# dohlee/rosettafold-pytorch

Hardware: AMD Instinct MI355X
Metric: residues/sec forward (L=256, N=128) (higher is better)
Workload: dtype bf16; 1 GPU; BASELINE.json configs[1]: bsz=4/GPU, n_seq=128, L=256, d_msa=384, d_pair=288, 8+5 blocks, 4 encoder layers, random-init weights; global_batch=4, parallelism=batch-sharded x1 (replicated weights), launch=one hipGraph replay per step (validation + input copy outside the graph)

## Files before the change

### include/rfmi.h

```cpp
#ifndef RFMI_H
#define RFMI_H
#include <stdint.h>

#ifdef __cplusplus
extern "C" {
#endif

#define RF_F32 0
#define RF_BF16 1
#define RF_F16 2
#define RF_F32X3 3

#define RF_EINVAL (-1)
#define RF_EALIGN (-2)

#define RF_ACT_NONE 0
#define RF_ACT_RELU 1
#define RF_ACT_ELU 2
#define RF_ACT_RELU_EPS 3
#define RF_ACT_LEAKY 4
#define RF_ACT_BLOCK_LN32 5

#define RF_BIAS_NONE 0
#define RF_BIAS_COL 1
// ... 93 lines not shown

int rf_outer_product_ln_linear(const void* xt, const void* yt, const void* wprime, const float* s, const float* c, float* out,
                               int B, int L, int N, int P, int Dout, float eps, const float* ln2_gamma, const float* ln2_beta,
                               float ln2_eps, void* y, int64_t y_ld, void* stream);

int rf_poswise(const void* q0, int q0_dtype, int64_t q0_ld, const void* k, int64_t k_ld, int k_col0, int k_hstride,
               int dlen, float* w, void* q_scale, int64_t qs_ld, int qs_col0, int qs_dh, int dtype, int B, int N, int L,
               int H, float scale, float qscale, void* stream);

int rf_weighted_msa_sum(const void* x, int dtype, const float* w, float* y, int64_t y_ld, int B, int N, int L, int D,
                        void* stream);

int64_t rf_instnorm_ws_bytes(int B, int64_t HW, int C);
int rf_instnorm_stats(const void* x, int x_dtype, void* sums , int B, int64_t HW, int C, void* workspace,
                      int64_t ws_bytes, void* stream);
int rf_instnorm_apply(const void* x, int x_dtype, const void* sums, const float* gamma, const float* beta, float eps,
                      const float* residual, int act, void* y, int y_dtype, void* y2, int y2_dtype, int B, int64_t HW,
                      int C, void* stream);

int rf_instnorm_mean(const void* sums, float* mean, int B, int64_t HW, int C, void* stream);
int64_t rf_channel_mean_ws_bytes(int B, int64_t HW, int C);
int rf_channel_mean(const float* x, float* mean, int B, int64_t HW, int C, void* workspace, int64_t ws_bytes, void* stream);
int rf_sample_mean(const void* x, int x_dtype, float* mean, int B, int64_t R, int C, int nsample, void* stream);
int rf_center_apply(const float* x, const float* mean, void* y, int y_dtype, int B, int64_t HW, int C, void* stream);
int rf_center_rows(float* x, float* mean, int B, int R, int C, void* stream);
int rf_fold_mean(const float* w, int64_t ldw, int k0, int K, int nseg, int64_t seg_stride, int sum_seg, const float* mean,
                 const float* bias, float* out, int B, int N, void* stream);
int rf_conv3x3_border_fix(void* y, int y_dtype, const float* taps, int B, int H, int W, int C, int dilation, int edges,
                          void* stream);

// ... 126 lines not shown
```

### rosettafold-pytorch_amd/_lib.py

```python
import ctypes as C
import os

import torch

_HERE = os.path.dirname(os.path.abspath(__file__))
LIB_PATH = os.environ.get("RFMI_LIB") or os.path.join(_HERE, "librfmi.so")

RF_F32, RF_BF16, RF_F16 = 0, 1, 2
RF_F32X3 = 3
ACT_NONE, ACT_RELU, ACT_ELU, ACT_RELU_EPS, ACT_LEAKY, ACT_BLOCK_LN32 = 0, 1, 2, 3, 4, 5
BIAS_NONE, BIAS_COL, BIAS_ROW = 0, 1, 2
AMODE_PLAIN, AMODE_CONV3X3 = 0, 1

i32, i64, f32, vp = C.c_int32, C.c_int64, C.c_float, C.c_void_p
u64 = C.c_uint64


class GemmDesc(C.Structure):
    _fields_ = [
        ("M", i32), ("N", i32), ("K", i32),
        ("nb0", i32), ("nb1", i32), ("nb2", i32),
        ("ab_dtype", i32), ("c_dtype", i32), ("kc", i32), ("a_mode", i32),
        ("a_rc", i32), ("b_rc", i32), ("c_rc", i32), ("c_cc", i32),
        ("a_bs", i64 * 3), ("a_ro", i64), ("a_ri", i64), ("a_ko", i64),
# ... 24 lines not shown
    "rf_tied_attention": [vp, vp, vp, C.POINTER(I64x4), C.POINTER(I64x4), vp, C.POINTER(I64x3), f32, vp, vp, i64, vp,
                          C.POINTER(I64x4), i32, i32, i32, i32, i32, vp, i64, vp],
    "rf_tied_softmax_ld": [vp, vp, i32, i64, vp, i64, i32, i32, i32, vp],
    "rf_tied_logits_ld": [vp, vp, C.POINTER(I64x4), vp, C.POINTER(I64x3), f32, vp, i64, vp, i64, i32, i32, i32, i32, i32, vp,
                          i64, vp],
    "rf_tied_av_ld": [vp, i64, vp, C.POINTER(I64x4), vp, C.POINTER(I64x4), i32, i32, i32, i32, i32, vp],
    "rf_tied_attention_ld": [vp, vp, vp, C.POINTER(I64x4), C.POINTER(I64x4), vp, C.POINTER(I64x3), f32, vp, i64, vp, i64, vp,
                             C.POINTER(I64x4), i32, i32, i32, i32, i32, vp, i64, vp],
    "rf_ffn_fused": [vp, i64, vp, vp, vp, vp, i64, vp, i64, vp, i64, vp, vp, f32, i64, i32, i32, vp],
    "rf_outer_product_ln_linear": [vp, vp, vp, vp, vp, vp, i32, i32, i32, i32, i32, f32, vp, vp, f32, vp, i64, vp],
    "rf_poswise_collapsed": [vp, vp, vp, i32, i32, i32, i32, i32, f32, vp],
    "rf_poswise": [vp, i32, i64, vp, i64, i32, i32, i32, vp, vp, i64, i32, i32, i32, i32, i32, i32, i32, f32, f32, vp],
    "rf_weighted_msa_sum": [vp, i32, vp, vp, i64, i32, i32, i32, i32, vp],
    "rf_instnorm_ws_bytes": [i32, i64, i32],
    "rf_instnorm_stats": [vp, i32, vp, i32, i64, i32, vp, i64, vp],
    "rf_instnorm_apply": [vp, i32, vp, vp, vp, f32, vp, i32, vp, i32, vp, i32, i32, i64, i32, vp],
    "rf_instnorm_mean": [vp, vp, i32, i64, i32, vp],
    "rf_channel_mean_ws_bytes": [i32, i64, i32],
    "rf_channel_mean": [vp, vp, i32, i64, i32, vp, i64, vp],
    "rf_sample_mean": [vp, i32, vp, i32, i64, i32, i32, vp],
    "rf_center_apply": [vp, vp, vp, i32, i32, i64, i32, vp],
    "rf_center_rows": [vp, vp, i32, i32, i32, vp],
    "rf_fold_mean": [vp, i64, i32, i32, i32, i64, i32, vp, vp, vp, i32, i32, vp],
    "rf_conv3x3_border_fix": [vp, i32, vp, i32, i32, i32, i32, i32, i32, vp],
    "rf_msa_embed": [vp, vp, vp, vp, vp, vp, i32, i32, i32, i32, vp],
    "rf_pair_embed": [vp, vp, vp, vp, vp, vp, vp, vp, i32, i32, i32, vp],
    "rf_copy4d": [vp, i32, C.POINTER(I64x4), vp, i32, C.POINTER(I64x4), C.POINTER(I64x4), vp],
    "rf_axpby": [vp, i32, f32, vp, i32, f32, vp, i32, i64, vp],
    "rf_favor_softmax_features": [vp, vp, C.POINTER(I64x4), i32, i32, vp, i32, i64, i32, i32, i32, i32, i32, i32, f32, vp],
    "rf_favor_attention": [vp, vp, vp, C.POINTER(I64x4), C.POINTER(I64x3), i32, i32, i32, i32, i32, i32, i32, i32, i32, i32, f32, vp],
# ... 109 lines not shown
```

### rosettafold-pytorch_amd/csrc/common.h

```cpp
#pragma once
#include <hip/hip_runtime.h>
#include <stdint.h>
#include <stdlib.h>

#include "rfmi.h"

typedef __attribute__((ext_vector_type(8))) short h16x8;
typedef __attribute__((ext_vector_type(4))) short h16x4;
typedef __attribute__((ext_vector_type(4))) float f32x4;
typedef unsigned short h16_t;
typedef __attribute__((ext_vector_type(2))) float rf_f32x2;

#define RF_WAVE 64

#ifdef RF_H16_IS_F16
#define RF_H16 RF_F16
#define RF_H16_ONE2 0x3C003C00u
typedef __attribute__((ext_vector_type(2))) _Float16 rf_h16x2;
typedef __attribute__((ext_vector_type(8))) _Float16 rf_h16x8n;
__device__ __forceinline__ float h2f(h16_t u) { return (float)__builtin_bit_cast(_Float16, u); }
__device__ __forceinline__ h16_t f2h(float x) { return __builtin_bit_cast(h16_t, (_Float16)x); }
__device__ __forceinline__ f32x4 rf_mfma16(h16x8 a, h16x8 b, f32x4 c, int, int, int) {
  return __builtin_amdgcn_mfma_f32_16x16x32_f16(__builtin_bit_cast(rf_h16x8n, a), __builtin_bit_cast(rf_h16x8n, b), c, 0, 0, 0);
}
// ... 119 lines not shown
  *out = v ? atoi(v) : 0;
  return 0;
}
#else
#define RF_DBG(x) 0
static inline int rf_dbg_env(const char* name, int* out) {
  *out = 0;
  return getenv(name) ? RF_EINVAL : 0;
}
#endif

static inline bool rf_env_flag(const char* name) { return getenv(name) != nullptr; }

int rf_gemm_fast_try(const rf_gemm_desc& d, int64_t batch, int* rc, void* stream);
int rf_gemm_wreg_try(const rf_gemm_desc& d, int64_t batch, int* rc, void* stream);
int rf_conv288_try(const rf_gemm_desc& d, int64_t batch, int* rc, void* stream);
void rf_gemm_fast_set_stamps(void* buf);
```

### rosettafold-pytorch_amd/csrc/conv288.hip

```cpp
#include <type_traits>

#include "common.h"

static __device__ __attribute__((aligned(16))) unsigned int g_conv_zero16[4];

struct Conv288P {
  const h16_t* x;
  const h16_t* w;
  const float* bias;
  h16_t* y;
  int B, H, W, dil;
  int tpr;
  int nt_store;
};

__global__ __launch_bounds__(512) void conv3x3_c288_kernel(const Conv288P p) {
  constexpr int C = 288, BM = 256, BN = 288;
  constexpr int WGN = 2, TM = 64, TN = 144, WM = 4, WN = 9;
  constexpr int A_PIECES = 17, B_PIECES = 18;
  constexpr int A_BYTES = A_PIECES * 1024, B_BYTES = B_PIECES * 1024;
  constexpr int SSTEP = A_BYTES + 3 * B_BYTES;
  constexpr int NPIECES = A_PIECES + 3 * B_PIECES;
  constexpr int PW = (NPIECES + 7) / 8;
  constexpr int NSS = 27;
  extern __shared__ __attribute__((aligned(16))) char smem[];
  const int tid = threadIdx.x, lane = tid & 63;
  const int wave = __builtin_amdgcn_readfirstlane(tid >> 6);
  const int wm = wave / WGN, wn = wave % WGN;
  const int fr = lane & 15, fq = lane >> 4;
// ... 77 lines not shown
    __builtin_amdgcn_s_barrier();
#pragma unroll
    for (int t = 0; t < PW; ++t) CONV_DMA(t)
    const unsigned sbase = (unsigned)((ss & 1) * SSTEP);
#include "conv288_schedule.inc"
  }
#undef CONV_RD
#undef CONV_RDA
#undef CONV_DMA

  __syncthreads();
  constexpr int PITCH = TN * 2 + 16;
  constexpr int CPR = TN * 2 / 16;
  constexpr int NIT = 32 * CPR / 64;
  char* const strip = smem + wave * (32 * PITCH);
  h16_t* const ytile = p.y + ((int64_t)row * p.W + j0) * C;
#pragma unroll
  for (int ip = 0; ip < 2; ++ip) {
#pragma unroll
    for (int ih = 0; ih < 2; ++ih)
#pragma unroll
      for (int j = 0; j < WN; ++j) {
        const f32x4 a = acc[ip * 2 + ih][j];
        uint2 o;
        o.x = rf_pack2_h16(a[0], a[1]);
        o.y = rf_pack2_h16(a[2], a[3]);
        *(uint2*)(strip + (ih * 16 + fr) * PITCH + (j * 16 + 4 * fq) * 2) = o;
      }
    asm volatile("" ::: "memory");
#pragma unroll
    for (int t = 0; t < NIT; ++t) {
      const int idx = lane + 64 * t;
      const int r = idx / CPR, c = idx % CPR;
      const f32x4 v = *(const f32x4*)(strip + r * PITCH + c * 16);
      f32x4* dst = (f32x4*)(ytile + (int64_t)(wm * TM + ip * 32 + r) * C + wn * TN + c * 8);
      if (p.nt_store)
        __builtin_nontemporal_store(v, dst);
      else
        *dst = v;
    }
    asm volatile("" ::: "memory");
  }
}

int rf_conv288_try(const rf_gemm_desc& d, int64_t batch, int* rc, void* stream) {
  *rc = 0;
  static const bool off = rf_env_flag("RF_NO_CONV288");
  if (off) return 0;
  if (d.a_mode != RF_AMODE_CONV3X3 || batch != 1 || d.ab_dtype != RF_H16 || d.c_dtype != RF_H16) return 0;
  if (d.conv_c != 288 || d.N != 288 || d.conv_w % 256 != 0 || d.conv_dil < 1 || d.conv_dil > 8) return 0;
  if (d.act != RF_ACT_NONE || d.alpha != 1.0f || d.residual || d.ln_out || d.c_rc > 0 || d.c_cc > 0 || d.c_ri != 288 || d.b_ri != 9 * 288)
    return 0;
  if (d.bias_mode != RF_BIAS_NONE && d.bias_mode != RF_BIAS_COL) return 0;
  if (((uintptr_t)d.A % 16) || ((uintptr_t)d.B % 16) || ((uintptr_t)d.C % 16) || (d.bias_mode == RF_BIAS_COL && ((uintptr_t)d.bias % 16))) return 0;
  Conv288P p;
  p.x = (const h16_t*)d.A; p.w = (const h16_t*)d.B; p.y = (h16_t*)d.C;
  p.bias = d.bias_mode == RF_BIAS_COL ? d.bias : nullptr;
  p.B = d.conv_n; p.H = d.conv_h; p.W = d.conv_w; p.dil = d.conv_dil;
  p.tpr = d.conv_w / 256;
  const int64_t nt = (int64_t)d.conv_n * d.conv_h * p.tpr;
  if (nt > 0x7fffffffLL) return 0;
  static const bool no_nt = rf_env_flag("RF_NO_NT_STORE");
  p.nt_store = ((int64_t)d.M * 288 * 2 > (64ll << 20)) && !no_nt;
  if (const int e = rf_enable_big_lds<conv3x3_c288_kernel>()) {
    *rc = e;
    return 1;
  }
  hipLaunchKernelGGL(conv3x3_c288_kernel, dim3((unsigned)nt), dim3(512), 2 * (17 + 54) * 1024, (hipStream_t)stream, p);
  *rc = rf_launch_status();
  return 1;
}
```

### rosettafold-pytorch_amd/csrc/gemm.hip

```cpp
#include <type_traits>

#include "common.h"

__device__ __attribute__((aligned(16))) unsigned int g_rf_zero16[4];

struct GemmP {
  rf_gemm_desc d;
  int tilesM, tilesN;
  int vec_store;
  int dbg;
  int stage_epi;
  int nt_store;
  int c_pow2, c_rsh, c_csh;
  int f32_vec;
  unsigned long long* stamps;
};

__device__ __forceinline__ int64_t split_off(int idx, int rc, int64_t ro, int64_t ri) {
  return rc > 0 ? (int64_t)(idx / rc) * ro + (int64_t)(idx % rc) * ri : (int64_t)idx * ri;
}

__device__ __forceinline__ void batch_decode(const rf_gemm_desc& d, int z, int& z0, int& z1, int& z2) {
  z2 = z % d.nb2;
  int t = z / d.nb2;
// ... 782 lines not shown
}

static unsigned long long* g_gemm_stamps = nullptr;
extern "C" int rf_debug_gemm_stamps(void* buf) {
  g_gemm_stamps = (unsigned long long*)buf;
  return 0;
}
extern "C" int rf_debug_gemm_fast_stamps(void* buf) {
  rf_gemm_fast_set_stamps(buf);
  return 0;
}

static thread_local int g_last_family = -1;
extern "C" int rf_gemm_last_family(void) { return g_last_family; }

extern "C" int rf_gemm(const rf_gemm_desc* dd, void* stream) {
  g_last_family = -1;
  if (!dd || !dd->A || !dd->B || !dd->C) return RF_EINVAL;
  GemmP p;
  p.d = *dd;
  p.dbg = (dd->tile_cfg >> 8) & 3;
#ifndef RF_ABLATION
  if (p.dbg) return RF_EINVAL;
#endif
  p.d.tile_cfg &= 0xff;
  rf_gemm_desc& d = p.d;
  if (d.M <= 0 || d.N <= 0 || d.K <= 0) return RF_EINVAL;
  if (d.alpha == 0.f || !__builtin_isfinite(d.alpha)) return RF_EINVAL;
  if (d.rs && (d.ab_dtype != RF_H16 || d.tile_cfg != 0 || d.rs_rpb <= 0 || d.rs_cg <= 0 || d.rs_cg % 16 || d.rs_ncols <= 0 ||
               d.rs_ncols % d.rs_cg))
    return RF_EINVAL;
// ... 96 lines not shown
  if (d.a_mode == RF_AMODE_CONV3X3) {
    if (d.conv_c % 8 != 0) return RF_EALIGN;
  } else if (!al8(d.a_ri) || !al8(d.a_ro) || !al8(d.a_ko) || !al8(d.a_bs[0]) || !al8(d.a_bs[1]) || !al8(d.a_bs[2])) {
    return RF_EALIGN;
  }
  if (!al8(d.b_ri) || !al8(d.b_ro) || !al8(d.b_ko) || !al8(d.b_bs[0]) || !al8(d.b_bs[1]) || !al8(d.b_bs[2]))
    return RF_EALIGN;

  if (want_ln) {
    if (d.c_dtype != RF_F32 || d.c_rc > 0 || d.c_cc > 0 || batch != 1 || !d.ln_gamma || !d.ln_beta ||
        ((uintptr_t)d.ln_out % 8) || ((uintptr_t)d.ln_gamma % 16) || ((uintptr_t)d.ln_beta % 16))
      return RF_EINVAL;
  }
  if (d.tile_cfg == 0 && !p.dbg && !p.stamps) {
    int rc = 0;
    if (d.a_mode == RF_AMODE_CONV3X3 && !want_ln && rf_conv288_try(d, batch, &rc, stream)) {
      g_last_family = 2;
      return rc;
    }
    if (rf_gemm_wreg_try(d, batch, &rc, stream)) {
      g_last_family = 4;
      return rc;
    }
    if (d.rs) return RF_EINVAL;
    if (rf_gemm_fast_try(d, batch, &rc, stream)) {
      g_last_family = 3;
      return rc;
    }
    if (want_ln) {
      rf_gemm_desc d2 = d;
      d2.ln_out = nullptr;
      if (rf_gemm_fast_try(d2, batch, &rc, stream)) {
// ... 43 lines not shown
  RF_CASE(64, 96, 64, 2, 2)
  RF_CASE(64, 96, 32, 2, 2)
  RF_CASE(64, 64, 64, 2, 2)
  RF_CASE(64, 64, 32, 2, 2)
  RF_CASE(256, 256, 64, 4, 2)
  RF_CASE(256, 288, 64, 4, 2)
  RF_CASE(256, 192, 64, 4, 2)
  RF_CASE(256, 128, 64, 4, 2)
  RF_CASE(256, 128, 32, 2, 2)
  RF_CASE(128, 256, 32, 2, 2)
#undef RF_CASE
  g_last_family = d.a_mode == RF_AMODE_CONV3X3 ? 2 : 1;
  if (rc != 0 || !want_ln) return rc;
  return rf_layernorm(d.C, RF_F32, d.c_ri, d.ln_out, RF_H16, d.N, d.M, d.N, d.ln_gamma, d.ln_beta, d.ln_eps, 1, RF_ACT_NONE, stream);
}
```

### rosettafold-pytorch_amd/csrc/ops.hip

```cpp
#include "common.h"

#define RF_CHECK_DT(dt) \
  if ((dt) != RF_F32 && (dt) != RF_H16) return RF_EINVAL

static inline unsigned cdiv(int64_t a, int64_t b) { return (unsigned)((a + b - 1) / b); }

static thread_local int g_last_route = -1;
extern "C" int rf_rowops_last_route(void) { return g_last_route; }

__device__ __forceinline__ float block_sum(float v, float* red) {
  v = wave_sum(v);
  const int w = threadIdx.x >> 6;
  __syncthreads();
  if ((threadIdx.x & 63) == 0) red[w] = v;
  __syncthreads();
  return red[0] + red[1] + red[2] + red[3];
}
__device__ __forceinline__ float block_max(float v, float* red) {
  v = wave_max(v);
  const int w = threadIdx.x >> 6;
  __syncthreads();
  if ((threadIdx.x & 63) == 0) red[w] = v;
  __syncthreads();
  return fmaxf(fmaxf(red[0], red[1]), fmaxf(red[2], red[3]));
// ... 681 lines not shown
  }
  __syncthreads();
  for (int c = threadIdx.x; c < 2 * C; c += 256) {
    float t = 0.f;
    for (int g = 0; g < ppi; ++g) t += sm[g * 2 * C + c];
    partials[((int64_t)b * gridDim.x + blockIdx.x) * 2 * C + c] = t;
  }
}

__global__ __launch_bounds__(256) void instnorm_finalize_kernel(const float* partials, double* sums, int nblk, int C) {
  __shared__ double part[8][32];
  const int b = blockIdx.y;
  const int cl = threadIdx.x & 31, g = threadIdx.x >> 5;
  const int c = blockIdx.x * 32 + cl;
  double t = 0.0;
  if (c < 2 * C)
    for (int k = g; k < nblk; k += 8) t += (double)partials[((int64_t)b * nblk + k) * 2 * C + c];
  part[g][cl] = t;
  __syncthreads();
  if (g == 0 && c < 2 * C) {
    double a = part[0][cl];
#pragma unroll
    for (int k = 1; k < 8; ++k) a += part[k][cl];
    sums[((int64_t)b * C + (c < C ? c : c - C)) * 2 + (c < C ? 0 : 1)] = a;
  }
}

__global__ __launch_bounds__(256) void instnorm_apply_vec_kernel(const h16_t* x, const double* sums, const float* gamma,
                                                                 const float* beta, float eps, const float* residual,
                                                                 int act, void* y, int y_dt, void* y2, int y2_dt,
                                                                 int64_t HW, int C) {
  extern __shared__ float sm[];
// ... 73 lines not shown
    const unsigned nblk = cdiv(HW, INV_PIX);
    const int ppi = 256 / (C / 8);
    hipLaunchKernelGGL(instnorm_stats_vec_kernel, dim3(nblk, B), dim3(256), (size_t)ppi * 2 * C * sizeof(float),
                       (hipStream_t)stream, (const h16_t*)x, (double*)sums, partials, HW, C);
    hipLaunchKernelGGL(instnorm_finalize_kernel, dim3(cdiv(2 * C, 32), B), dim3(256), 0, (hipStream_t)stream, partials,
                       (double*)sums, (int)nblk, C);
    g_last_route = 31;
    return rf_launch_status();
  }
  const unsigned nblk = cdiv(HW, IN_PIX);
  hipLaunchKernelGGL(instnorm_stats_kernel, dim3(nblk, B), dim3(256), 0, (hipStream_t)stream, x, x_dtype, (double*)sums,
                     partials, HW, C);
  hipLaunchKernelGGL(instnorm_finalize_kernel, dim3(cdiv(2 * C, 32), B), dim3(256), 0, (hipStream_t)stream, partials,
                     (double*)sums, (int)nblk, C);
  g_last_route = 30;
  return rf_launch_status();
}

__global__ __launch_bounds__(256) void instnorm_apply_kernel(const void* x, int x_dt, const double* sums,
                                                             const float* gamma, const float* beta, float eps,
                                                             const float* residual, int act, void* y, int y_dt,
                                                             void* y2, int y2_dt, int64_t HW, int C, int64_t total) {
  for (int64_t e = (int64_t)blockIdx.x * 256 + threadIdx.x; e < total; e += (int64_t)gridDim.x * 256) {
    const int c = e % C;
    const int64_t b = e / (HW * C);
    const double s = sums[(b * C + c) * 2], q = sums[(b * C + c) * 2 + 1];
    const double mean = s / (double)HW;
    double var = q / (double)HW - mean * mean;
    var = var > 0.0 ? var : 0.0;
    float v = gamma ? (ld(x, x_dt, e) - (float)mean) * rsqrtf((float)var + eps) * gamma[c] + beta[c] : ld(x, x_dt, e) - (float)mean;
// ... 627 lines not shown
      p = pe[aa_idx[b * L + l] * D + c];
    y[e] = x[e] + p;
  }
}

extern "C" int rf_add_pos_enc(const float* x, const int64_t* aa_idx, const float* pe, float* y, int B, int N, int L, int D,
                              int two_d, void* stream) {
  if (two_d && (N != L || D % 2)) return RF_EINVAL;
  const int64_t total = (int64_t)B * N * L * D;
  if (total <= 0) return RF_EINVAL;
  hipLaunchKernelGGL(add_pos_enc_kernel, dim3(min(cdiv(total, 256), 16384u)), dim3(256), 0, (hipStream_t)stream, x, aa_idx, pe,
                     y, N, L, D, two_d, total);
  return rf_launch_status();
}

extern "C" int rf_version(void) { return 14; }
#ifdef RF_H16_IS_F16
extern "C" const char* rf_build_info(void) { return "librfmi_f16 gfx950 (MI355X) round-3: 16-bit operand type = IEEE fp16"; }
#else
extern "C" const char* rf_build_info(void) { return "librfmi gfx950 (MI355X) round-3: 16-bit operand type = bfloat16"; }
#endif
extern "C" int rf_h16_dtype(void) { return RF_H16; }
```

### rosettafold-pytorch_amd/model.py

```python
import math
from collections import namedtuple

import torch
import torch.nn as nn

from . import _lib as L
from . import ops
from .ops import F32
from .runtime import RT, T, manual_seed, dropout_, _f, fresh_f32
from .backward import (_RecordedFn, _recording, _check_backward_call, _copy, _dropout_rec, _replay_dropout,
                       _grad_scale, _scaled_copy, _unscale, _conv_weight_grad, _param_grads, _pre_norm_residual_bwd,
                       conv_input_grad_weight, conv3x3_input_grad)

N_IDX, CA_IDX, C_IDX = 0, 1, 2
M_FEAT = 266
M_PAD = 288
VT_ROWS = 80
_SeqGeometry = namedtuple("_SeqGeometry", "B Ls Lo ss so RB R S W2 ctx_scale")


def set_compute_dtype(dtype):
    if dtype not in (torch.bfloat16, torch.float16, torch.float32):
        raise TypeError("compute dtype must be bfloat16, float16 or float32")
    RT.dtype = dtype
# ... 1212 lines not shown
        blk = self.resnet[1].fn
        cond = RT.condition and ops.is_h16(T()) and Dp % 4 == 0
        bias = _f(self.resnet[0].bias)
        if cond:
            bias_b = self._center_1d(msa1d, bias)
        ops.tile_1d_feats(msa1d, feat, Kf, Dp, B, Lr, 2 * P)
        ln(self.ln_pair, pair, out=feat, out_ld=Kf, out_off=Dp + 4 * P)
        ops.copy4d(att.contiguous(), (0, 0, H, 1), feat, (0, 0, Kf, 1), (1, 1, B * Lr * Lr, H), y_off=2 * Dp + 4 * P)
        if cond:
            x = torch.empty(B, Lr, Lr, Dp, device=dev, dtype=F32)
            for b in range(B):
                ops.linear(feat[b], self.wt("f", self.resnet[0], kpad=Kf), bias_b[b], out=x[b])
            cx = ops.sample_mean(x)
            y = conv3x3(self, "c1", blk[1], ops.center_apply(x, cx, out_dtype=T()), 1)
            ops.conv3x3_border_fix(y, self._conv_taps(blk[1], cx), 1)
        else:
            x = ops.linear(feat, self.wt("f", self.resnet[0], kpad=Kf), bias, out_dtype=F32)
            y = conv3x3(self, "c1", blk[1], ops.cast(x, T()), 1)
        y, _ = ops.instnorm(y, _f(blk[2].weight), _f(blk[2].bias), eps=blk[2].eps, act=L.ACT_ELU, out_dtype=T())
        if self.training:
            dropout_(y, _p(blk[4]))
        y = conv3x3(self, "c2", blk[5], y, 1)
        out, _ = ops.instnorm(y, _f(blk[6].weight), _f(blk[6].bias), eps=blk[6].eps, residual=x, act=L.ACT_ELU,
                              out_dtype=F32)
        return out

    def forward(self, msa, pair, att):
        return self.run(msa.float().contiguous(), pair.float().contiguous(), att.float().contiguous())


def conv3x3(mod, key, conv, x, dilation, out_dtype=None):
    B, Hh, Ww, Cc = x.shape
    Co = conv.weight.shape[0]
    wk = mod.cached(("conv", key), lambda: conv.weight.detach().permute(0, 2, 3, 1).reshape(Co, 9 * Cc).to(T()).contiguous())
    out = torch.empty(B, Hh, Ww, Co, device=x.device, dtype=out_dtype or T())
    ops.gemm(x, wk, out, B * Hh * Ww, Co, 9 * Cc, conv=(B, Hh, Ww, Cc, dilation),
             bias=_f(conv.bias) if conv.bias is not None else None)
    return out


class PairUpdateWithAxialAttentionLayer(RecordingModule):
    _rf_scales_own_grads = True

    def __init__(self, d_pair, d_ff, n_heads, p_dropout, performer_kws):
        super().__init__()
        self.row_attn = PerformerSelfAttention(dim=d_pair, heads=n_heads, dropout=p_dropout,
                                               generalized_attention=True, **performer_kws)
        self.col_attn = PerformerSelfAttention(dim=d_pair, heads=n_heads, dropout=p_dropout,
                                               generalized_attention=True, **performer_kws)
        self.ff = FeedForward(d_pair, d_ff, p_dropout)
        self.layer = nn.Sequential(
            Residual(nn.Sequential(LayerNorm(d_pair), RowWise(self.row_attn))),
            Residual(nn.Sequential(LayerNorm(d_pair), ColWise(self.col_attn))),
# ... 404 lines not shown
        nxt = shard.haloed_buffer(h, W, y.shape[-1], next_halo, x_t.device, T())
        o_f, o_t = ops.instnorm(shard.interior(y, d), _f(f[5].weight), _f(f[5].bias), eps=f[5].eps, residual=x_f, act=L.ACT_ELU,
                                out_dtype=F32, out2=shard.interior(nxt, next_halo), **kw)
        return o_t, o_f

    def run(self, x_t, x_f, row_group=None, rows_global=None, next_halo=0, tape=None):
        f = self.layer.fn
        kw = {} if row_group is None else {"row_group": row_group, "rows_global": rows_global}
        _check_backward_call(self, tape, row_group, x_t.shape[-1])
        rec = tape is not None
        if row_group is not None and x_t.shape[0] == 1:
            return self._run_rows_b1(x_t, x_f, row_group, rows_global, next_halo)

        def conv(key, c, x):
            if row_group is None:
                return conv3x3(self, key, c, x, self.dilation)
            from . import shard
            xh = shard.exchange_row_halos(x, self.dilation, row_group)
            return shard.drop_row_halos(conv3x3(self, key, c, xh, self.dilation), self.dilation)

        stats = [] if rec else None
        y = conv("c1", f[0], x_t)
        if rec:
            tape.update(x_t=x_t, y1=y)
        y, _ = ops.instnorm(y, _f(f[1].weight), _f(f[1].bias), eps=f[1].eps, act=L.ACT_ELU, out_dtype=T(), stats_out=stats, **kw)
        p = _p(f[3]) if self.training else 0.0
        if rec:
            tape["a1"] = _copy(y) if p > 0 else y
            tape["drop"] = _dropout_rec(y, p)
            tape["a1d"] = y
        else:
            dropout_(y, p)
        y = conv("c2", f[4], y)
        o_f, o_t = ops.instnorm(y, _f(f[5].weight), _f(f[5].bias), eps=f[5].eps, residual=x_f, act=L.ACT_ELU,
                                out_dtype=F32, out2_dtype=T(), stats_out=stats, **kw)
        if rec:
            tape.update(y2=y, s1=stats[0], s2=stats[1], o_f=o_f)
        return o_t, o_f

    def _backward(self, tape, g):
        f, d = self.layer.fn, self.dilation
        dy2, dg5, db5 = ops.instnorm_bwd(g, tape["y2"], tape["s2"], _f(f[5].weight), eps=f[5].eps, act_out=tape["o_f"],
                                         dx_dtype=T(), ge_out=g)
        dw2, _ = ops.conv_wgrad(dy2, tape["a1d"], 9, d)
        da = conv3x3_input_grad(self, "c2", f[4], dy2, d)
        _replay_dropout(da, tape["drop"])
        dy1, dg1, db1 = ops.instnorm_bwd(da, tape["y1"], tape["s1"], _f(f[1].weight), eps=f[1].eps, act_out=tape["a1"],
                                         dx_dtype=T())
        dw1, _ = ops.conv_wgrad(dy1, tape["x_t"], 9, d)
        dx = conv3x3_input_grad(self, "c1", f[0], dy1, d, residual=g)
# ... 177 lines not shown
```

### rosettafold-pytorch_amd/ops.py

```python
import ctypes as C

import torch

from . import _lib as L
from ._lib import lib, check, GemmDesc, I64x4, I64x3

F32, BF16, F16 = torch.float32, torch.bfloat16, torch.float16
_H16_CODE = {torch.bfloat16: L.RF_BF16, torch.float16: L.RF_F16}
_H16_TORCH = {L.RF_BF16: torch.bfloat16, L.RF_F16: torch.float16}


def is_h16(dtype):
    return dtype in _H16_CODE


def h16():
    return _H16_TORCH[L.active_h16()]


def dcode(dtype):
    if dtype == torch.float32:
        return L.RF_F32
    code = _H16_CODE.get(dtype)
    if code is None:
# ... 42 lines not shown
            raise L.RfmiError("librfmi ops need device tensors (there is no CPU fallback)")
        if dev is None:
            dev = t.device
        elif t.device != dev:
            raise L.RfmiError(f"operands on different devices: {dev} and {t.device}")
    if dev is not None and dev.index != torch.cuda.current_device():
        raise L.RfmiError(f"operands live on {dev} but the current device is cuda:{torch.cuda.current_device()} "
                          "(wrap the call in torch.cuda.device(...))")


def gemm(A, B, Cout, M, N, K, *, batch=(1, 1, 1), a_off=0, b_off=0, c_off=0,
         a_bs=(0, 0, 0), a_row=(0, 0, None), a_ko=0,
         b_bs=(0, 0, 0), b_row=(0, 0, None), b_ko=0, kc=0,
         c_bs=(0, 0, 0), c_row=(0, 0, None), c_col=(0, 0),
         bias=None, bias_mode=None, act=L.ACT_NONE, act_nvalid=0, act_eps=0.0, alpha=1.0,
         residual=None, res_off=None, conv=None, tile_cfg=0, ln=None, block_ln=None, rs=None, exact=False):
    _need_cuda(A, B, Cout, bias, residual)
    if A.dtype != B.dtype:
        raise TypeError("A and B dtypes differ")
    d = GemmDesc()
    d.M, d.N, d.K = int(M), int(N), int(K)
    d.nb0, d.nb1, d.nb2 = [int(x) for x in batch]
    d.ab_dtype, d.c_dtype = gemm_code(A.dtype, exact), dcode(Cout.dtype)
    d.kc = int(kc)
    d.a_rc, d.a_ro, d.a_ri = int(a_row[0]), int(a_row[1]), int(K if a_row[2] is None else a_row[2])
    d.b_rc, d.b_ro, d.b_ri = int(b_row[0]), int(b_row[1]), int(K if b_row[2] is None else b_row[2])
    d.c_rc, d.c_ro, d.c_ri = int(c_row[0]), int(c_row[1]), int(N if c_row[2] is None else c_row[2])
    d.c_cc, d.c_co = int(c_col[0]), int(c_col[1])
    for i in range(3):
        d.a_bs[i], d.b_bs[i], d.c_bs[i] = int(a_bs[i]), int(b_bs[i]), int(c_bs[i])
    d.a_ko, d.b_ko = int(a_ko), int(b_ko)
# ... 16 lines not shown
        d.residual = residual.data_ptr() + (c_off if res_off is None else res_off) * 4
    if block_ln is not None:
        g, b, eps = block_ln
        _need_cuda(g, b)
        d.ln_gamma, d.ln_beta, d.ln_eps = g.data_ptr(), b.data_ptr(), float(eps)
    if rs is not None:
        t_, bstride, rpb, cg, ncols, alpha_ = rs
        _need_cuda(t_)
        if t_.dtype != F32:
            raise TypeError("rs must be fp32")
        d.rs, d.rs_bstride, d.rs_rpb, d.rs_cg, d.rs_ncols, d.rs_alpha = t_.data_ptr(), int(bstride), int(rpb), int(cg), int(ncols), float(alpha_)
    if ln is not None:
        ln_out, g, b, eps = ln
        _need_cuda(ln_out, g, b)
        d.ln_out, d.ln_gamma, d.ln_beta, d.ln_eps = ln_out.data_ptr(), g.data_ptr(), b.data_ptr(), float(eps)
    check(lib.rf_gemm(C.byref(d), stream()), "rf_gemm")
    return Cout


_NO_WREG = bool(int(__import__("os").environ.get("RF_NO_WREG_GEMM", "0") or "0"))


def gemm_takes_row_scale(M, N, K):
    return (not _NO_WREG) and K in (288, 384) and M % 64 == 0 and M >= 16384 and N % 128 == 0 and N >= 256


def linear(x, w, bias=None, *, out=None, out_dtype=None, act=L.ACT_NONE, residual=None, alpha=1.0, tile_cfg=0, ln=None,
           exact=False):
    K = x.shape[-1]
    Mrows = x.numel() // K
    N = w.shape[0]
    if w.shape[1] != K:
# ... 222 lines not shown

def poswise(q0, q0_ld, k, k_ld, k_col0, k_hs, dlen, w, q_scale, qs_ld, qs_col0, qs_dh, B, N, L_, H, scale, qscale):
    _need_cuda(q0, k, w, q_scale)
    check(lib.rf_poswise(ptr(q0), dcode(q0.dtype), q0_ld, ptr(k), k_ld, k_col0, k_hs, dlen, ptr(w), ptr(q_scale),
                         qs_ld, qs_col0, qs_dh, dcode(k.dtype), B, N, L_, H, scale, qscale, stream()), "rf_poswise")


def weighted_msa_sum(x, w, y, y_ld):
    B, N, L_, D = x.shape
    _need_cuda(x, w, y)
    check(lib.rf_weighted_msa_sum(ptr(x), dcode(x.dtype), ptr(w), ptr(y), y_ld, B, N, L_, D, stream()),
          "rf_weighted_msa_sum")


def instnorm(x, gamma, beta, *, eps=1e-6, residual=None, act=L.ACT_NONE, out_dtype=None, out2_dtype=None, row_group=None,
             rows_global=None, out=None, out2=None, stats_out=None):
    B, H, W, Cc = x.shape
    _need_cuda(x, gamma, beta, residual)
    sums = torch.empty(B * Cc * 2, device=x.device, dtype=torch.float64)
    ws_bytes = int(lib.rf_instnorm_ws_bytes(B, H * W, Cc))
    ws = torch.empty(ws_bytes, device=x.device, dtype=torch.uint8)
    check(lib.rf_instnorm_stats(ptr(x), dcode(x.dtype), ptr(sums), B, H * W, Cc, ptr(ws), ws_bytes, stream()),
          "rf_instnorm_stats")
    if row_group is not None:
        from . import shard
        shard.all_reduce_sum(sums, row_group)
        sums.mul_(float(H) / float(rows_global))
    if stats_out is not None:
        stats_out.append(sums)
    y = out if out is not None else torch.empty(x.shape, device=x.device, dtype=out_dtype or x.dtype)
    y2 = out2 if out2 is not None else (torch.empty(x.shape, device=x.device, dtype=out2_dtype) if out2_dtype is not None else None)
    for t in (y, y2):
        if t is not None and (tuple(t.shape) != tuple(x.shape) or not t.is_contiguous()):
            raise ValueError("instnorm: out / out2 must be contiguous tensors of the input's shape")
    _need_cuda(y, y2)
    check(lib.rf_instnorm_apply(ptr(x), dcode(x.dtype), ptr(sums), ptr(gamma), ptr(beta), eps, ptr(residual), act,
                                ptr(y), dcode(y.dtype), ptr(y2), dcode(y2.dtype) if y2 is not None else 0, B, H * W,
                                Cc, stream()), "rf_instnorm_apply")
# ... 605 lines not shown
```

### rosettafold-pytorch_amd/runtime.py

```python
import torch

from . import ops
from .ops import F32


class _Runtime:
    dtype = torch.bfloat16
    f32_precision = "highest"
    train_seed = 0
    train_offset = 0
    cache_epoch = 0
    struct_inputs_fp32 = True
    head_center = bool(int(__import__("os").environ.get("RF_HEAD_CENTER", "1")))
    condition = bool(int(__import__("os").environ.get("RF_CONDITION", "1")))
    condition_values = bool(int(__import__("os").environ.get("RF_CONDITION_V", "1")))
    se3_fused_radial = not bool(int(__import__("os").environ.get("RF_SE3_UNFUSED", "0")))
    fused_favor = True
    fused_outer_ln = not bool(int(__import__("os").environ.get("RF_NO_FUSED_OUTER_LN", "0")))
    fused_tied = not bool(int(__import__("os").environ.get("RF_NO_FUSED_TIED", "0")))
    fused_outer = not bool(int(__import__("os").environ.get("RF_NO_FUSED_OUTER", "0")))
    outer_bwd_slab_bytes = int(float(__import__("os").environ.get("RF_OUTER_BWD_SLAB_MB", "6")) * (1 << 20))
    outer_bwd_fused = not bool(int(__import__("os").environ.get("RF_NO_FUSED_OUTER_BWD", "0")))
    tied_v2 = not bool(int(__import__("os").environ.get("RF_TIED_V1", "0")))
    tied_fold_w = not bool(int(__import__("os").environ.get("RF_TIED_NO_FOLD", "0")))
    rowshard_attention = __import__("os").environ.get("RF_ROWSHARD_ATTENTION", "transpose")


RT = _Runtime()

# ... 30 lines not shown
```

Baseline: 3211 residues/s.

## Fuse instance-norm statistics into the conv3x3 C=288 GEMM epilogue

The conv3x3 kernel for 288 channels now computes per-channel sum and sum-of-squares in its epilogue. It rounds the values to 16 bits first, reduces them across lanes with DPP, then across waves in LDS, and writes one partial row per block. A finalize kernel turns these partials into the fp64 sums that instnorm takes, so the separate stats pass over the conv output is skipped in the pair ResNet blocks. The finalize reduction loop is also unrolled by eight to raise load parallelism. The cost is extra epilogue work, LDS use and a workspace write per conv block, and instnorm falls back to the old stats pass when the fused kernel is not chosen.

After: 3204 residues/s. Within noise of the previous version (-0.2%).

```diff
diff --git a/include/rfmi.h b/include/rfmi.h
--- a/include/rfmi.h
+++ b/include/rfmi.h
@@ -131,6 +131,7 @@
 int64_t rf_instnorm_ws_bytes(int B, int64_t HW, int C);
 int rf_instnorm_stats(const void* x, int x_dtype, void* sums , int B, int64_t HW, int C, void* workspace,
                       int64_t ws_bytes, void* stream);
+int rf_conv3x3_instnorm_stats(const rf_gemm_desc* d, void* sums, void* workspace, int64_t ws_bytes, void* stream);
 int rf_instnorm_apply(const void* x, int x_dtype, const void* sums, const float* gamma, const float* beta, float eps,
                       const float* residual, int act, void* y, int y_dtype, void* y2, int y2_dtype, int B, int64_t HW,
                       int C, void* stream);
diff --git a/rosettafold-pytorch_amd/_lib.py b/rosettafold-pytorch_amd/_lib.py
--- a/rosettafold-pytorch_amd/_lib.py
+++ b/rosettafold-pytorch_amd/_lib.py
@@ -62,6 +62,7 @@
     "rf_weighted_msa_sum": [vp, i32, vp, vp, i64, i32, i32, i32, i32, vp],
     "rf_instnorm_ws_bytes": [i32, i64, i32],
     "rf_instnorm_stats": [vp, i32, vp, i32, i64, i32, vp, i64, vp],
+    "rf_conv3x3_instnorm_stats": [vp, vp, vp, i64, vp],
     "rf_instnorm_apply": [vp, i32, vp, vp, vp, f32, vp, i32, vp, i32, vp, i32, i32, i64, i32, vp],
     "rf_instnorm_mean": [vp, vp, i32, i64, i32, vp],
     "rf_channel_mean_ws_bytes": [i32, i64, i32],
diff --git a/rosettafold-pytorch_amd/csrc/common.h b/rosettafold-pytorch_amd/csrc/common.h
--- a/rosettafold-pytorch_amd/csrc/common.h
+++ b/rosettafold-pytorch_amd/csrc/common.h
@@ -157,5 +157,6 @@
 
 int rf_gemm_fast_try(const rf_gemm_desc& d, int64_t batch, int* rc, void* stream);
 int rf_gemm_wreg_try(const rf_gemm_desc& d, int64_t batch, int* rc, void* stream);
-int rf_conv288_try(const rf_gemm_desc& d, int64_t batch, int* rc, void* stream);
+int rf_conv288_try(const rf_gemm_desc& d, int64_t batch, int* rc, void* stream, float* partials);
+int rf_instnorm_finalize(const float* partials, void* sums, int B, int nblk, int C, void* stream);
 void rf_gemm_fast_set_stamps(void* buf);
diff --git a/rosettafold-pytorch_amd/csrc/conv288.hip b/rosettafold-pytorch_amd/csrc/conv288.hip
--- a/rosettafold-pytorch_amd/csrc/conv288.hip
+++ b/rosettafold-pytorch_amd/csrc/conv288.hip
@@ -12,7 +12,13 @@
   int B, H, W, dil;
   int tpr;
   int nt_store;
+  float* partials;
 };
+
+template <int CTRL>
+__device__ __forceinline__ float conv_dpp_add(float v) {
+  return v + __builtin_bit_cast(float, __builtin_amdgcn_update_dpp(0, __builtin_bit_cast(int, v), CTRL, 0xf, 0xf, false));
+}
 
 __global__ __launch_bounds__(512) void conv3x3_c288_kernel(const Conv288P p) {
   constexpr int C = 288, BM = 256, BN = 288;
@@ -120,6 +126,34 @@
   constexpr int CPR = TN * 2 / 16;
   constexpr int NIT = 32 * CPR / 64;
   char* const strip = smem + wave * (32 * PITCH);
+  float* const red = (float*)(smem + 8 * (32 * PITCH));
+  if (p.partials) {
+#pragma unroll
+    for (int j = 0; j < WN; ++j) {
+      f32x4 s = {0.f, 0.f, 0.f, 0.f}, q = {0.f, 0.f, 0.f, 0.f};
+#pragma unroll
+      for (int ii = 0; ii < WM; ++ii) {
+        const f32x4 a = acc[ii][j];
+        const unsigned lo = rf_pack2_h16(a[0], a[1]), hi = rf_pack2_h16(a[2], a[3]);
+        const f32x4 v = {rf_h16_lo(lo), rf_h16_hi(lo), rf_h16_lo(hi), rf_h16_hi(hi)};
+#pragma unroll
+        for (int e = 0; e < 4; ++e) {
+          s[e] += v[e];
+          q[e] = fmaf(v[e], v[e], q[e]);
+        }
+      }
+#pragma unroll
+      for (int e = 0; e < 4; ++e) {
+        s[e] = conv_dpp_add<0x140>(conv_dpp_add<0x141>(conv_dpp_add<0x4e>(conv_dpp_add<0xb1>(s[e]))));
+        q[e] = conv_dpp_add<0x140>(conv_dpp_add<0x141>(conv_dpp_add<0x4e>(conv_dpp_add<0xb1>(q[e]))));
+      }
+      if (fr == 0) {
+        float* const r = red + wm * 2 * C + wn * TN + j * 16 + 4 * fq;
+        *(f32x4*)r = s;
+        *(f32x4*)(r + C) = q;
+      }
+    }
+  }
   h16_t* const ytile = p.y + ((int64_t)row * p.W + j0) * C;
 #pragma unroll
   for (int ip = 0; ip < 2; ++ip) {
@@ -147,9 +181,14 @@
     }
     asm volatile("" ::: "memory");
   }
+  if (p.partials) {
+    __syncthreads();
+    float* const pp = p.partials + (int64_t)lid * 2 * C;
+    for (int c = tid; c < 2 * C; c += 512) pp[c] = ((red[c] + red[2 * C + c]) + red[4 * C + c]) + red[6 * C + c];
+  }
 }
 
-int rf_conv288_try(const rf_gemm_desc& d, int64_t batch, int* rc, void* stream) {
+int rf_conv288_try(const rf_gemm_desc& d, int64_t batch, int* rc, void* stream, float* partials) {
   *rc = 0;
   static const bool off = rf_env_flag("RF_NO_CONV288");
   if (off) return 0;
@@ -168,6 +207,7 @@
   if (nt > 0x7fffffffLL) return 0;
   static const bool no_nt = rf_env_flag("RF_NO_NT_STORE");
   p.nt_store = ((int64_t)d.M * 288 * 2 > (64ll << 20)) && !no_nt;
+  p.partials = partials;
   if (const int e = rf_enable_big_lds<conv3x3_c288_kernel>()) {
     *rc = e;
     return 1;
diff --git a/rosettafold-pytorch_amd/csrc/gemm.hip b/rosettafold-pytorch_amd/csrc/gemm.hip
--- a/rosettafold-pytorch_amd/csrc/gemm.hip
+++ b/rosettafold-pytorch_amd/csrc/gemm.hip
@@ -820,7 +820,7 @@
 static thread_local int g_last_family = -1;
 extern "C" int rf_gemm_last_family(void) { return g_last_family; }
 
-extern "C" int rf_gemm(const rf_gemm_desc* dd, void* stream) {
+static int gemm_dispatch(const rf_gemm_desc* dd, void* stream, float* conv_partials, bool* conv_partials_used) {
   g_last_family = -1;
   if (!dd || !dd->A || !dd->B || !dd->C) return RF_EINVAL;
   GemmP p;
@@ -947,8 +947,9 @@
   }
   if (d.tile_cfg == 0 && !p.dbg && !p.stamps) {
     int rc = 0;
-    if (d.a_mode == RF_AMODE_CONV3X3 && !want_ln && rf_conv288_try(d, batch, &rc, stream)) {
+    if (d.a_mode == RF_AMODE_CONV3X3 && !want_ln && rf_conv288_try(d, batch, &rc, stream, conv_partials)) {
       g_last_family = 2;
+      if (conv_partials_used) *conv_partials_used = conv_partials != nullptr;
       return rc;
     }
     if (rf_gemm_wreg_try(d, batch, &rc, stream)) {
@@ -1022,3 +1023,19 @@
   if (rc != 0 || !want_ln) return rc;
   return rf_layernorm(d.C, RF_F32, d.c_ri, d.ln_out, RF_H16, d.N, d.M, d.N, d.ln_gamma, d.ln_beta, d.ln_eps, 1, RF_ACT_NONE, stream);
 }
+
+extern "C" int rf_gemm(const rf_gemm_desc* dd, void* stream) { return gemm_dispatch(dd, stream, nullptr, nullptr); }
+
+extern "C" int rf_conv3x3_instnorm_stats(const rf_gemm_desc* d, void* sums, void* workspace, int64_t ws_bytes, void* stream) {
+  if (!d || !sums || !d->C || d->a_mode != RF_AMODE_CONV3X3 || d->conv_n <= 0 || d->conv_h <= 0 || d->conv_w <= 0 || d->N <= 0)
+    return RF_EINVAL;
+  if (d->nb0 > 1 || d->nb1 > 1 || d->nb2 > 1 || d->c_rc > 0 || d->c_cc > 0 || d->c_ri != d->N) return RF_EINVAL;
+  const int B = d->conv_n, C = d->N;
+  const int64_t HW = (int64_t)d->conv_h * d->conv_w;
+  if (!workspace || ws_bytes < rf_instnorm_ws_bytes(B, HW, C)) return RF_EINVAL;
+  bool used = false;
+  const int rc = gemm_dispatch(d, stream, (float*)workspace, &used);
+  if (rc != 0) return rc;
+  if (used) return rf_instnorm_finalize((const float*)workspace, sums, B, (int)(HW / 256), C, stream);
+  return rf_instnorm_stats(d->C, d->c_dtype, sums, B, HW, C, workspace, ws_bytes, stream);
+}
diff --git a/rosettafold-pytorch_amd/csrc/ops.hip b/rosettafold-pytorch_amd/csrc/ops.hip
--- a/rosettafold-pytorch_amd/csrc/ops.hip
+++ b/rosettafold-pytorch_amd/csrc/ops.hip
@@ -719,8 +719,18 @@
   const int cl = threadIdx.x & 31, g = threadIdx.x >> 5;
   const int c = blockIdx.x * 32 + cl;
   double t = 0.0;
-  if (c < 2 * C)
-    for (int k = g; k < nblk; k += 8) t += (double)partials[((int64_t)b * nblk + k) * 2 * C + c];
+  if (c < 2 * C) {
+    const float* const col = partials + (int64_t)b * nblk * 2 * C + c;
+    int k = g;
+    for (; k + 56 < nblk; k += 64) {
+      float v[8];
+#pragma unroll
+      for (int u = 0; u < 8; ++u) v[u] = col[(int64_t)(k + 8 * u) * 2 * C];
+#pragma unroll
+      for (int u = 0; u < 8; ++u) t += (double)v[u];
+    }
+    for (; k < nblk; k += 8) t += (double)col[(int64_t)k * 2 * C];
+  }
   part[g][cl] = t;
   __syncthreads();
   if (g == 0 && c < 2 * C) {
@@ -824,6 +834,13 @@
   hipLaunchKernelGGL(instnorm_finalize_kernel, dim3(cdiv(2 * C, 32), B), dim3(256), 0, (hipStream_t)stream, partials,
                      (double*)sums, (int)nblk, C);
   g_last_route = 30;
+  return rf_launch_status();
+}
+
+int rf_instnorm_finalize(const float* partials, void* sums, int B, int nblk, int C, void* stream) {
+  hipLaunchKernelGGL(instnorm_finalize_kernel, dim3(cdiv(2 * C, 32), B), dim3(256), 0, (hipStream_t)stream, partials,
+                     (double*)sums, nblk, C);
+  g_last_route = -1;
   return rf_launch_status();
 }
 
@@ -1481,7 +1498,7 @@
   return rf_launch_status();
 }
 
-extern "C" int rf_version(void) { return 14; }
+extern "C" int rf_version(void) { return 15; }
 #ifdef RF_H16_IS_F16
 extern "C" const char* rf_build_info(void) { return "librfmi_f16 gfx950 (MI355X) round-3: 16-bit operand type = IEEE fp16"; }
 #else
diff --git a/rosettafold-pytorch_amd/model.py b/rosettafold-pytorch_amd/model.py
--- a/rosettafold-pytorch_amd/model.py
+++ b/rosettafold-pytorch_amd/model.py
@@ -1250,29 +1250,32 @@
             cx = ops.sample_mean(x)
             y = conv3x3(self, "c1", blk[1], ops.center_apply(x, cx, out_dtype=T()), 1)
             ops.conv3x3_border_fix(y, self._conv_taps(blk[1], cx), 1)
+            s1 = None
         else:
             x = ops.linear(feat, self.wt("f", self.resnet[0], kpad=Kf), bias, out_dtype=F32)
-            y = conv3x3(self, "c1", blk[1], ops.cast(x, T()), 1)
-        y, _ = ops.instnorm(y, _f(blk[2].weight), _f(blk[2].bias), eps=blk[2].eps, act=L.ACT_ELU, out_dtype=T())
+            y, s1 = conv3x3(self, "c1", blk[1], ops.cast(x, T()), 1, stats=True)
+        y, _ = ops.instnorm(y, _f(blk[2].weight), _f(blk[2].bias), eps=blk[2].eps, act=L.ACT_ELU, out_dtype=T(), sums=s1)
         if self.training:
             dropout_(y, _p(blk[4]))
-        y = conv3x3(self, "c2", blk[5], y, 1)
+        y, s2 = conv3x3(self, "c2", blk[5], y, 1, stats=True)
         out, _ = ops.instnorm(y, _f(blk[6].weight), _f(blk[6].bias), eps=blk[6].eps, residual=x, act=L.ACT_ELU,
-                              out_dtype=F32)
+                              out_dtype=F32, sums=s2)
         return out
 
     def forward(self, msa, pair, att):
         return self.run(msa.float().contiguous(), pair.float().contiguous(), att.float().contiguous())
 
 
-def conv3x3(mod, key, conv, x, dilation, out_dtype=None):
+def conv3x3(mod, key, conv, x, dilation, out_dtype=None, stats=False):
     B, Hh, Ww, Cc = x.shape
     Co = conv.weight.shape[0]
     wk = mod.cached(("conv", key), lambda: conv.weight.detach().permute(0, 2, 3, 1).reshape(Co, 9 * Cc).to(T()).contiguous())
     out = torch.empty(B, Hh, Ww, Co, device=x.device, dtype=out_dtype or T())
-    ops.gemm(x, wk, out, B * Hh * Ww, Co, 9 * Cc, conv=(B, Hh, Ww, Cc, dilation),
-             bias=_f(conv.bias) if conv.bias is not None else None)
-    return out
+    bias = _f(conv.bias) if conv.bias is not None else None
+    if stats and RT.conv_stats:
+        return out, ops.conv3x3_instnorm_stats(x, wk, out, dilation, bias)
+    ops.gemm(x, wk, out, B * Hh * Ww, Co, 9 * Cc, conv=(B, Hh, Ww, Cc, dilation), bias=bias)
+    return (out, None) if stats else out
 
 
 class PairUpdateWithAxialAttentionLayer(RecordingModule):
@@ -1707,16 +1710,17 @@
 
         def conv(key, c, x):
             if row_group is None:
-                return conv3x3(self, key, c, x, self.dilation)
+                return conv3x3(self, key, c, x, self.dilation, stats=True)
             from . import shard
             xh = shard.exchange_row_halos(x, self.dilation, row_group)
-            return shard.drop_row_halos(conv3x3(self, key, c, xh, self.dilation), self.dilation)
+            return shard.drop_row_halos(conv3x3(self, key, c, xh, self.dilation), self.dilation), None
 
         stats = [] if rec else None
-        y = conv("c1", f[0], x_t)
+        y, sums = conv("c1", f[0], x_t)
         if rec:
             tape.update(x_t=x_t, y1=y)
-        y, _ = ops.instnorm(y, _f(f[1].weight), _f(f[1].bias), eps=f[1].eps, act=L.ACT_ELU, out_dtype=T(), stats_out=stats, **kw)
+        y, _ = ops.instnorm(y, _f(f[1].weight), _f(f[1].bias), eps=f[1].eps, act=L.ACT_ELU, out_dtype=T(), stats_out=stats,
+                            sums=sums, **kw)
         p = _p(f[3]) if self.training else 0.0
         if rec:
             tape["a1"] = _copy(y) if p > 0 else y
@@ -1724,9 +1728,9 @@
             tape["a1d"] = y
         else:
             dropout_(y, p)
-        y = conv("c2", f[4], y)
+        y, sums = conv("c2", f[4], y)
         o_f, o_t = ops.instnorm(y, _f(f[5].weight), _f(f[5].bias), eps=f[5].eps, residual=x_f, act=L.ACT_ELU,
-                                out_dtype=F32, out2_dtype=T(), stats_out=stats, **kw)
+                                out_dtype=F32, out2_dtype=T(), stats_out=stats, sums=sums, **kw)
         if rec:
             tape.update(y2=y, s1=stats[0], s2=stats[1], o_f=o_f)
         return o_t, o_f
diff --git a/rosettafold-pytorch_amd/ops.py b/rosettafold-pytorch_amd/ops.py
--- a/rosettafold-pytorch_amd/ops.py
+++ b/rosettafold-pytorch_amd/ops.py
@@ -80,7 +80,7 @@
          b_bs=(0, 0, 0), b_row=(0, 0, None), b_ko=0, kc=0,
          c_bs=(0, 0, 0), c_row=(0, 0, None), c_col=(0, 0),
          bias=None, bias_mode=None, act=L.ACT_NONE, act_nvalid=0, act_eps=0.0, alpha=1.0,
-         residual=None, res_off=None, conv=None, tile_cfg=0, ln=None, block_ln=None, rs=None, exact=False):
+         residual=None, res_off=None, conv=None, tile_cfg=0, ln=None, block_ln=None, rs=None, exact=False, conv_sums=None):
     _need_cuda(A, B, Cout, bias, residual)
     if A.dtype != B.dtype:
         raise TypeError("A and B dtypes differ")
@@ -127,8 +127,21 @@
         ln_out, g, b, eps = ln
         _need_cuda(ln_out, g, b)
         d.ln_out, d.ln_gamma, d.ln_beta, d.ln_eps = ln_out.data_ptr(), g.data_ptr(), b.data_ptr(), float(eps)
+    if conv_sums is not None:
+        ws_bytes = int(lib.rf_instnorm_ws_bytes(d.conv_n, d.conv_h * d.conv_w, d.N))
+        ws = torch.empty(ws_bytes, device=Cout.device, dtype=torch.uint8)
+        check(lib.rf_conv3x3_instnorm_stats(C.byref(d), ptr(conv_sums), ptr(ws), ws_bytes, stream()), "rf_conv3x3_instnorm_stats")
+        return Cout
     check(lib.rf_gemm(C.byref(d), stream()), "rf_gemm")
     return Cout
+
+
+def conv3x3_instnorm_stats(x, wk, out, dilation, bias=None):
+    B, H, W, Cc = x.shape
+    Co = wk.shape[0]
+    sums = torch.empty(B * Co * 2, device=x.device, dtype=torch.float64)
+    gemm(x, wk, out, B * H * W, Co, 9 * Cc, conv=(B, H, W, Cc, dilation), bias=bias, conv_sums=sums)
+    return sums
 
 
 _NO_WREG = bool(int(__import__("os").environ.get("RF_NO_WREG_GEMM", "0") or "0"))
@@ -381,14 +394,17 @@
 
 
 def instnorm(x, gamma, beta, *, eps=1e-6, residual=None, act=L.ACT_NONE, out_dtype=None, out2_dtype=None, row_group=None,
-             rows_global=None, out=None, out2=None, stats_out=None):
+             rows_global=None, out=None, out2=None, stats_out=None, sums=None):
     B, H, W, Cc = x.shape
-    _need_cuda(x, gamma, beta, residual)
-    sums = torch.empty(B * Cc * 2, device=x.device, dtype=torch.float64)
-    ws_bytes = int(lib.rf_instnorm_ws_bytes(B, H * W, Cc))
-    ws = torch.empty(ws_bytes, device=x.device, dtype=torch.uint8)
-    check(lib.rf_instnorm_stats(ptr(x), dcode(x.dtype), ptr(sums), B, H * W, Cc, ptr(ws), ws_bytes, stream()),
-          "rf_instnorm_stats")
+    _need_cuda(x, gamma, beta, residual, sums)
+    if sums is None:
+        sums = torch.empty(B * Cc * 2, device=x.device, dtype=torch.float64)
+        ws_bytes = int(lib.rf_instnorm_ws_bytes(B, H * W, Cc))
+        ws = torch.empty(ws_bytes, device=x.device, dtype=torch.uint8)
+        check(lib.rf_instnorm_stats(ptr(x), dcode(x.dtype), ptr(sums), B, H * W, Cc, ptr(ws), ws_bytes, stream()),
+              "rf_instnorm_stats")
+    elif sums.dtype != torch.float64 or sums.numel() != B * Cc * 2 or not sums.is_contiguous():
+        raise ValueError("instnorm: sums must be the contiguous fp64 [B * C * 2] of rf_instnorm_stats")
     if row_group is not None:
         from . import shard
         shard.all_reduce_sum(sums, row_group)
diff --git a/rosettafold-pytorch_amd/runtime.py b/rosettafold-pytorch_amd/runtime.py
--- a/rosettafold-pytorch_amd/runtime.py
+++ b/rosettafold-pytorch_amd/runtime.py
@@ -13,6 +13,7 @@
     struct_inputs_fp32 = True
     head_center = bool(int(__import__("os").environ.get("RF_HEAD_CENTER", "1")))
     condition = bool(int(__import__("os").environ.get("RF_CONDITION", "1")))
+    conv_stats = bool(int(__import__("os").environ.get("RF_CONV_STATS", "1")))
     condition_values = bool(int(__import__("os").environ.get("RF_CONDITION_V", "1")))
     se3_fused_radial = not bool(int(__import__("os").environ.get("RF_SE3_UNFUSED", "0")))
     fused_favor = True
```
